# Genesis-Embodied-AI/ThinShellLab

Measured on AMD Instinct MI355X. Metric: element-steps/s (fwd+adjoint), 100k-tri cloth; 1/2/4/8-GPU scaling, higher is better.
Workload: dtype f64

## Files before the change

### thinshelllab_amd/csrc/k_cloth.hpp

```cpp
#pragma once
#include "tsl_ctx.hpp"
#include "tsl_device.hpp"

struct FaceGeom {
  d3 n;
  double h[3];
  double ca[3];
};

TSL_DEV FaceGeom face_geom(const d3 P[3]) {
  FaceGeom g;
  g.n = normalized(cross(P[1] - P[0], P[2] - P[1]));
#pragma unroll
  for (int l = 0; l < 3; l++) {
    const d3 p = P[l], a = P[(l + 1) % 3], b = P[(l + 2) % 3];
    const d3 en = cross(g.n, b - a);
    g.h[l] = fabs(dot(p - a, en)) / norm(en);
    g.ca[l] = dot(normalized(a - p), normalized(b - p));
  }
  return g;
}

TSL_DEV bool sign_neg(const d3& n2, const d3& e) { return dot(n2, e) < -1e-10 * norm(e); }
TSL_DEV double dihedral(const d3& n1, const d3& n2, const d3& e) {
// ... 384 lines not shown
            if (l != m) L[(m * 3 + j) * 9 + l * 3 + k] += Hlm[k * 3 + j];
          }
      }
  }

  if (CLAMP_ALL) spd_clamp<9>(L);
  double* R = rec + (size_t)t * 81;
#pragma unroll
  for (int l = 0; l < 3; l++)
#pragma unroll
    for (int m = 0; m < 3; m++)
#pragma unroll
      for (int j = 0; j < 3; j++)
#pragma unroll
        for (int k = 0; k < 3; k++) R[(l * 3 + m) * 9 + j * 3 + k] = L[(l * 3 + j) * 9 + m * 3 + k];
}

__global__ void __launch_bounds__(256) k_cloth_hess_hinge(ClothArgs A, const double* __restrict__ pos, double* __restrict__ rec) {
  const int h = blockIdx.x * blockDim.x + threadIdx.x;
  if (h >= A.n_hinge) return;
  const int f1 = A.hg_info[8 * h], l = A.hg_info[8 * h + 1], f2 = A.hg_info[8 * h + 2], p4 = A.hg_info[8 * h + 3], p21 = A.hg_info[8 * h + 4];
  const ClothDev c = A.cloth[A.cid[f1]];
  int v1[3], v2[3]; d3 P1[3], P2[3];
  load_face(pos, A.f2v, f1, v1, P1);
  load_face(pos, A.f2v, f2, v2, P2);
  const FaceGeom g1 = face_geom(P1), g2 = face_geom(P2);
  d3 g[4];
  hinge_grad(g1, g2, l, p4, p21, g);
  const double d2 = 2.0 * c.Kb * c.dx * c.dx * (1.0 / 3.0);
  double* R = rec + (size_t)h * 16;
#pragma unroll
  for (int j = 0; j < 4; j++) { R[3 * j] = g[j].x; R[3 * j + 1] = g[j].y; R[3 * j + 2] = g[j].z; }
  R[12] = d2;
}

#define CG_BPW 28
__global__ void __launch_bounds__(256) k_cloth_gather(int n_blk, const int* __restrict__ base, const int* __restrict__ ptr, const unsigned* __restrict__ ent, int n_hinge, int n_cface,
                                                      const double* __restrict__ hrec, const double* __restrict__ frec, const double* __restrict__ trec, double* __restrict__ vals) {
  __shared__ double tile[9][CG_BPW + 1];
  const int b0 = blockIdx.x * CG_BPW, t = threadIdx.x;
  if (t < 9 * CG_BPW) {
    const int bl = t / 9, e9 = t - 9 * bl, b = b0 + bl, r = e9 / 3, c = e9 - 3 * r;
    double acc = 0.0;
    if (b < n_blk) {
      for (int q = ptr[b]; q < ptr[b + 1]; q++) {
        const unsigned e = ent[q];
        const int el = (int)((e >> 4) & 0x7ffffff), pr = (int)(e & 15);
        if ((e >> 30) == 1) {
          acc += trec[(size_t)(el & 0x3ffffff) * 144 + pr * 9 + e9];
        } else if (e >> 31) {
          const int j = pr >> 2, k = pr & 3;
          const double* R = hrec + (size_t)el * 16;
          acc += R[12] * (R[3 * j + r] * R[3 * k + c]);
        } else {
          acc += frec[(size_t)el * 81 + pr * 9 + e9];
        }
      }
    }
    tile[e9][bl] = acc;
  }
  __syncthreads();
  if (t < 9 * CG_BPW) {
    const int e9 = t / CG_BPW, bl = t - CG_BPW * e9, b = b0 + bl;
    if (b < n_blk) vals[(size_t)base[b] + 64 * e9] += tile[e9][bl];
  }
}
// ... 14 lines not shown
```

### thinshelllab_amd/csrc/k_contact.hpp

```cpp
#pragma once

#include "k_solver.hpp"
#include "tsl_ctx.hpp"
#include "tsl_device.hpp"

struct ContactArgs {
  const int* idx;
  const double *w, *n, *dx0, *k, *mu, *T;
  double k_contact, eps_contact, eps_vh;
};

TSL_DEV double fr_f0(double x, double eh) { return (x > eh) ? x : (-x * x * x / (3.0 * eh * eh) + x * x / eh + eh / 3.0); }
TSL_DEV double fr_f1(double x, double eh) { return (x > eh) ? 1.0 / x : (-x / (eh * eh) + 2.0 / eh); }
TSL_DEV double fr_f2(double x, double eh) { return (x > eh) ? -1.0 / (x * x) : -1.0 / (eh * eh); }

__global__ void k_vn_gather(int NV, const int* __restrict__ ptr, const int* __restrict__ lst, const int* __restrict__ faces, const double* __restrict__ pos, double* __restrict__ vn) {
  const int i = blockIdx.x * blockDim.x + threadIdx.x;
  if (i >= NV) return;
  d3 a = d3();
  for (int e = ptr[i]; e < ptr[i + 1]; e++) {
    const int f = lst[e];
    const d3 v1 = ld3(pos, faces[3 * f]), v2 = ld3(pos, faces[3 * f + 1]), v3 = ld3(pos, faces[3 * f + 2]);
    a = a + cross(v2 - v1, v3 - v1);
  }
// ... 462 lines not shown

#define CONTACT_MV_THREADS 1024
TSL_DEV double contact_matvec_lane(int nc, const int* __restrict__ idx, const int* __restrict__ rowpos, const double* __restrict__ Hm, const double* __restrict__ x,
                                   double* __restrict__ y) {
  const int ci = blockIdx.x * 64 + (threadIdx.x >> 4);
  const int r = threadIdx.x & 15;
  if (ci >= nc || r >= 12) return 0.0;
  const double* H = Hm + 144 * (size_t)ci + 12 * r;
  double s = 0, xr = 0;
  int prr = 0;
#pragma unroll
  for (int k = 0; k < 4; k++) {
    const int pk = rowpos[idx[4 * ci + k]];
    const d3 v = ld3(x, pk);
    s += H[3 * k] * v.x + H[3 * k + 1] * v.y + H[3 * k + 2] * v.z;
    if (k == r / 3) { prr = pk; xr = (r % 3 == 0) ? v.x : (r % 3 == 1) ? v.y : v.z; }
  }
  if (s != 0.0) atomicAdd(&y[3 * (size_t)prr + (r % 3)], s);
  return s * xr;
}

__global__ void k_cr_count(int nc, const int* __restrict__ idx, const int* __restrict__ rowpos, int* __restrict__ cnt) {
  const int q = blockIdx.x * blockDim.x + threadIdx.x;
  if (q >= 4 * nc) return;
  atomicAdd(&cnt[rowpos[idx[q]]], 1);
}
__global__ void k_cr_fill(int nc, const int* __restrict__ idx, const int* __restrict__ rowpos, const int* __restrict__ ptr, int* __restrict__ fill, int* __restrict__ tmp) {
  const int q = blockIdx.x * blockDim.x + threadIdx.x;
  if (q >= 4 * nc) return;
  const int p = rowpos[idx[q]];
  tmp[ptr[p] + atomicAdd(&fill[p], 1)] = q;
}
__global__ void k_cr_rank(int nc, const int* __restrict__ idx, const int* __restrict__ rowpos, const int* __restrict__ ptr, const int* __restrict__ tmp, int* __restrict__ ent,
                          int4* __restrict__ rows) {
  const int q = blockIdx.x * blockDim.x + threadIdx.x;
  if (q >= 4 * nc) return;
  const int c4 = q & ~3;
  const int4 r = make_int4(rowpos[idx[c4]], rowpos[idx[c4 + 1]], rowpos[idx[c4 + 2]], rowpos[idx[c4 + 3]]);
  const int p = (q & 3) == 0 ? r.x : (q & 3) == 1 ? r.y : (q & 3) == 2 ? r.z : r.w;
  const int s0 = ptr[p], s1 = ptr[p + 1];
  int rank = 0;
  for (int e = s0; e < s1; e++) rank += tmp[e] < q ? 1 : 0;
  ent[s0 + rank] = q;
  rows[s0 + rank] = r;
}

__global__ void __launch_bounds__(CONTACT_MV_THREADS)
k_contact_matvec(int nc, const int* __restrict__ idx, const int* __restrict__ rowpos, const double* __restrict__ Hm, const double* __restrict__ x,
                 double* __restrict__ y, CgScal* sc, int slot, int check_flag) {
  if (check_flag && sc->flag) return;
  double acc = contact_matvec_lane(nc, idx, rowpos, Hm, x, y);
  if (slot >= 0) {
    acc = wave_sum(acc);
    if ((threadIdx.x & 63) == 0 && acc != 0.0) atomicAdd(&sc->pAp[slot], acc);
  }
}



__global__ void k_contact_backprop(int nc, ContactArgs A, const double* __restrict__ pos, const double* __restrict__ z, double* __restrict__ cg) {
  const int ci = blockIdx.x * blockDim.x + threadIdx.x;
  if (ci >= nc) return;
  int id[4];
  for (int k = 0; k < 4; k++) id[k] = A.idx[4 * ci + k];
  const d3 x0 = ld3(pos, id[0]), xa = ld3(pos, id[1]), xb = ld3(pos, id[2]), xp = ld3(pos, id[3]);
  const double w[3] = {A.w[3 * ci], A.w[3 * ci + 1], A.w[3 * ci + 2]};
  const double kf = A.k[ci];
  const double* T = A.T + 6 * (size_t)ci;
  const d3 x_c = x0 * w[0] + xa * w[1] + xb * w[2];
  const d3 dx = xp - x_c - ld3(A.dx0, ci);
  const double u[2] = {T[0] * dx.x + T[1] * dx.y + T[2] * dx.z, T[3] * dx.x + T[4] * dx.y + T[5] * dx.z};
  const double r = sqrt(u[0] * u[0] + u[1] * u[1]);
  const double f1 = fr_f1(r, A.eps_vh), f2 = fr_f2(r, A.eps_vh);
  const double pressure = kf / A.mu[ci];
  double g1[3];
  for (int j = 0; j < 3; j++) g1[j] = kf * f1 * (u[0] * T[j] + u[1] * T[3 + j]);
  const d3 n_c = ld3(A.n, ci);
// ... 566 lines not shown
    HIP_OK(hipMemcpyAsync(&n_ee, c->ee_qscan.p + QE, sizeof(int), hipMemcpyDeviceToHost, s));
    HIP_OK(hipMemcpyAsync(&big_edges, c->ee_nvf.p + 1, sizeof(int), hipMemcpyDeviceToHost, s));
  }
  int nc = 0, big_bucket = 0;
  if (Q > 0) HIP_OK(hipMemcpyAsync(&nc, c->cq_scan.p + Q, sizeof(int), hipMemcpyDeviceToHost, s));
  HIP_OK(hipMemcpyAsync(&big_bucket, c->nc_dev.p + 1, sizeof(int), hipMemcpyDeviceToHost, s));
  HIP_OK(hipStreamSynchronize(s));
  HIP_OK(hipGetLastError());
  if (big_bucket > 0) {
    c->nc = 0;
    return tsl_fail("contact detection: %d triangles of one body fall into one broad-phase cell (more than %d are not ranked): the body lies outside grid_extent = %g m "
                    "(centroids are clamped into the boundary cells) or grid_h = %g m is far larger than its triangles", big_bucket, TSL_BUCKET_CAP, c->grid_extent, c->grid_h);
  }
  if (big_edges > 0) {
    c->nc = 0;
    return tsl_fail("contact detection (contact_ee): %d surface-edge midpoints of one body fall into one broad-phase cell (more than %d are not ranked): the body lies "
                    "outside grid_extent = %g m or grid_h = %g m is far larger than its edges", big_edges, TSL_BUCKET_CAP, c->grid_extent, c->grid_h);
  }
  if (ee && (long)nc + n_ee > c->max_n_constraints) {
    c->nc = 0;
    return tsl_fail("contact detection: %d vertex-triangle + %d edge-edge active constraints exceed max_n_constraints = %d (raise the scene's max_n_constraints)", nc, n_ee,
                    c->max_n_constraints);
  }
  if (nc > c->max_n_constraints) {
    c->nc = 0;
    return tsl_fail("contact detection: %d active constraints exceed max_n_constraints = %d (raise the scene's max_n_constraints)", nc, c->max_n_constraints);
  }
  nc += n_ee;
  c->nc = nc; c->nc_ee = n_ee;
  if (nc_host) *nc_host = c->nc;
  if (c->nc > 0) {
    const int n1 = NV + 1;
    if (c->cr_ptr.n == 0) {
      if (c->cr_ptr.alloc(n1) | c->cr_cnt.alloc(n1) | c->cr_fill.alloc(n1) | c->cr_ent.alloc(4 * (size_t)c->max_n_constraints) | c->cr_rows.alloc(4 * (size_t)c->max_n_constraints) | c->cr_tmp.alloc(4 * (size_t)c->max_n_constraints)) return -1;
    }
    HIP_OK(hipMemsetAsync(c->cr_cnt.p, 0, n1 * sizeof(int), s));
    HIP_OK(hipMemsetAsync(c->cr_fill.p, 0, n1 * sizeof(int), s));
    hipLaunchKernelGGL(k_cr_count, dim3(cnblk(4 * (long)c->nc, 256)), dim3(256), 0, s, c->nc, c->c_idx.p, c->rowpos.p, c->cr_cnt.p);
    scan_exclusive(s, n1, c->cr_cnt.p, c->cr_ptr.p, c->scan_tmp.p);
    hipLaunchKernelGGL(k_cr_fill, dim3(cnblk(4 * (long)c->nc, 256)), dim3(256), 0, s, c->nc, c->c_idx.p, c->rowpos.p, (const int*)c->cr_ptr.p, c->cr_fill.p, c->cr_tmp.p);
    hipLaunchKernelGGL(k_cr_rank, dim3(cnblk(4 * (long)c->nc, 256)), dim3(256), 0, s, c->nc, c->c_idx.p, c->rowpos.p, (const int*)c->cr_ptr.p, (const int*)c->cr_tmp.p, c->cr_ent.p, c->cr_rows.p);
    HIP_OK(hipGetLastError());
  }
  return 0;
}

static ContactArgs ee_args(ContactArgs A, int nvf) {
  A.idx += 4 * (size_t)nvf; A.w += 3 * (size_t)nvf; A.n += 3 * (size_t)nvf; A.dx0 += 3 * (size_t)nvf; A.k += nvf; A.mu += nvf; A.T += 6 * (size_t)nvf;
  return A;
}

extern "C" int tsl_contact_counts(tsl_ctx* c, int32_t* out2) {
  if (!c || !out2) return tsl_fail("tsl_contact_counts: null argument");
  out2[0] = c->nc - c->nc_ee; out2[1] = c->nc_ee;
  return 0;
}

static bool direct_takes_solve(tsl_ctx* c);
static void contact_diag_refresh(tsl_ctx* c, hipStream_t s) {
  hipLaunchKernelGGL(k_contact_diag, dim3(cnblk((long)c->NV * 64, 256)), dim3(256), 0, s, c->NV, (const int*)c->cr_ptr.p, (const int*)c->cr_ent.p, (const double*)c->c_H.p, c->c_diag.p);
  c->cdiag_valid = true;
}
static int contact_assemble(tsl_ctx* c, const double* pos, int spd, double* grad, hipStream_t s) {
  if (c->nc <= 0) return 0;
  ContactArgs A;
  A.idx = c->c_idx.p; A.w = c->c_w.p; A.n = c->c_n.p; A.dx0 = c->c_dx0.p; A.k = c->c_k.p; A.mu = c->c_mu.p; A.T = c->c_T.p;
  A.k_contact = c->k_contact; A.eps_contact = c->eps_contact; A.eps_vh = c->eps_v * c->dt;
  if (grad && c->c_G.n < 12 * (size_t)c->max_n_constraints) { if (c->c_G.alloc(12 * (size_t)c->max_n_constraints)) return -1; }
  double* cg = grad ? c->c_G.p : (double*)nullptr;
  const int nvf = c->nc - c->nc_ee;
  if (nvf > 0) {
    if (c->spd_literal && spd == 1) hipLaunchKernelGGL(k_contact_assemble_coop<true>, dim3(cnblk((long)nvf * 16, 256)), dim3(256), 0, s, nvf, A, pos, spd, c->c_Hfull.p, cg);
    else hipLaunchKernelGGL(k_contact_assemble_coop<false>, dim3(cnblk((long)nvf * 16, 256)), dim3(256), 0, s, nvf, A, pos, spd, c->c_Hfull.p, cg);
  }
// ... 64 lines not shown
```

### thinshelllab_amd/csrc/tsl_ctx.hpp

```cpp
#pragma once
#include <memory>
#include <hip/hip_runtime.h>
#include <stdint.h>

#include <algorithm>
#include <cmath>
#include <cstdio>
#include <cstring>
#include <string>
#include <vector>

#include "../../include/tsl_hip.h"
#include "k_body.hpp"
#include "direct_plan.hpp"

#define TSL_SLICE 64

extern thread_local std::string g_tsl_err;
int tsl_fail(const char* fmt, ...);

#define HIP_OK(call)                                                                     \
  do {                                                                                   \
    hipError_t e__ = (call);                                                             \
    if (e__ != hipSuccess) return tsl_fail("%s failed: %s (%s:%d)", #call, hipGetErrorString(e__), __FILE__, __LINE__); \
// ... 259 lines not shown
  bool pc_separate = false, pc_frozen = false, in_step = false;
  bool cdiag_valid = false;
  bool dinv_valid = false;
  const double *st_pos = nullptr, *st_prev = nullptr, *st_vel = nullptr, *st_ref = nullptr;
  int fwd_spd_pc = 1;
  int adj_spd_pc = 1;
  DevBuf<SolverScalars> scal;
  DevBuf<double> part_pAp, part_rz, part_rr;
  SolverScalars* h_scal = nullptr;
  SolverScalars* h_scal2 = nullptr;
  hipEvent_t rb_event[2] = {nullptr, nullptr};
  hipStream_t side = 0;
  hipEvent_t ev_fork = nullptr, ev_fork0 = nullptr, ev_g2 = nullptr, ev_join = nullptr, ev_join2 = nullptr, ev_hh = nullptr, ev_gf = nullptr;
  hipStream_t side2 = 0;

  DevBuf<double> F, pdir, x1;

  int n_body = 0, n_pair = 0;
  std::vector<tsl_body> h_bodies;
  std::vector<tsl_contact_pair> h_pairs;
  std::vector<int> self_contact;
  DevBuf<int> faces;
  DevBuf<int> border;
  DevBuf<double> vn;
  DevBuf<int> proj_flag, proj_dir, proj_idx;
  DevBuf<double> proj_w;
  DevBuf<int> nc_dev;
  int nc = 0;
  DevBuf<int> c_idx;
  DevBuf<double> c_w, c_n, c_dx0, c_k, c_mu, c_T;
  DevBuf<int> cr_ptr, cr_cnt, cr_fill, cr_ent;
  DevBuf<int4> cr_rows;
  DevBuf<int> cr_tmp;
  DevBuf<int> c_kind;
  DevBuf<double> c_H;
  DevBuf<double> c_Hfull;
  DevBuf<double> c_diag;
  DevBuf<double> c_G;
  DevBuf<int> grid_key, grid_val, grid_key2, grid_val2, grid_range;
  DevBuf<int> vnf_ptr, vnf_lst;
  DevBuf<int> cq_flag, cq_scan;
  DevBuf<int> grid_scan;
  std::vector<size_t> gb_f0, gb_t0, gb_s0;
  DevBuf<int> grid_cnt, grid_ptr, grid_cur, scan_tmp;
  int grid_buckets_max = 0;
  int max_body_faces = 0;
  struct EeDesc { int pair, target, qoff, nq; };
  int contact_ee = 0, nc_ee = 0;
  std::vector<int> h_ee_e0;
  std::vector<EeDesc> ee_desc;
  std::vector<char> ee_target;
  long ee_qtot = 0;
  bool ee_ready = false;
  DevBuf<int> ee_edges, ee_qlist;
  DevBuf<int> ee_key, ee_val, ee_key2, ee_val2, ee_range, ee_bcnt, ee_bptr, ee_bcur, ee_bscan;
  std::vector<size_t> ee_f0, ee_t0, ee_s0;
  DevBuf<unsigned long long> ee_lmax;
  DevBuf<int> ee_qcnt, ee_qscan, ee_cand, ee_scan_tmp, ee_nvf;

  std::vector<MgCloth*> mg;
  int mg_enable = -1;
  double mg_omega = 0.0;
  int mg_pi_iters = 12;
  DevBuf<double> mg_omega0, mg_pi_part, mg_pi_norm;
  int mg_nu = 1, mg_coarse_sweeps = 8, mg_fuse = 1, mg_fuse_restrict = 1, mg_max_levels = 16, mg_coarse_exact = 1, mg_coarse_lag = 0, mg_dense_nodes = 64, mg_dense_auto = 1;
  double last_step_iters_per_solve = 0.0;
// ... 36 lines not shown
```

### thinshelllab_amd/csrc/tsl_hip.hip

```cpp
#include <stdarg.h>
#include <cctype>
#include <chrono>
#include <mutex>

#include <array>
#include <map>

#include "k_cloth.hpp"
#include "k_contact.hpp"
#include "k_fem.hpp"
#include "k_mg.hpp"
#include "k_param.hpp"
#include "k_solver.hpp"
#include "tsl_ctx.hpp"

thread_local std::string g_tsl_err;
int tsl_fail(const char* fmt, ...) {
  char buf[1024];
  va_list ap;
  va_start(ap, fmt);
  vsnprintf(buf, sizeof(buf), fmt, ap);
  va_end(ap);
  g_tsl_err = buf;
  return -1;
// ... 564 lines not shown
  hipStream_t s = c->stream;
  if (c->n_cface) hipLaunchKernelGGL(k_cloth_normals, dim3(nblk(c->n_cface, 256)), dim3(256), 0, s, c->n_cface, pos, c->cf_f2v.p, c->norm_dir.p);
  const int nmax = std::max(std::max(c->NV, c->n_cface), std::max(c->n_hinge, c->n_tet));
  const int nvf = c->nc - c->nc_ee;
  const int nb1 = nblk(nmax, 256), nb2 = nvf > 0 ? nblk(nvf, 64) : 0, nb3 = c->nc_ee > 0 ? nblk(c->nc_ee, 64) : 0;
  if (c->e_part.n < (size_t)nb1 + (size_t)nblk(c->max_n_constraints, 64) + 1) { if (c->e_part.alloc((size_t)nb1 + (size_t)nblk(c->max_n_constraints, 64) + 1)) return -1; }
  if (c->n_stvk > 0) hipLaunchKernelGGL(k_energy_stvk, dim3(nb1), dim3(256), 0, s, vert_args(c), cloth_args(c), tet_args(c), pos, prev, vel, ref, c->e_part.p, stvk_args(c));
  else hipLaunchKernelGGL(k_energy, dim3(nb1), dim3(256), 0, s, vert_args(c), cloth_args(c), tet_args(c), pos, prev, vel, ref, c->e_part.p);
  if (nb2 > 0) hipLaunchKernelGGL(k_contact_energy, dim3(nb2), dim3(64), 0, s, nvf, contact_args(c), pos, c->e_part.p + nb1);
  if (nb3 > 0) hipLaunchKernelGGL(k_ee_energy, dim3(nb3), dim3(64), 0, s, c->nc_ee, ee_args(contact_args(c), nvf), pos, c->e_part.p + nb1 + nb2);
  hipLaunchKernelGGL(k_energy_final, dim3(1), dim3(256), 0, s, nb1 + nb2 + nb3, (const double*)c->e_part.p, &SC(c)->energy);
  return 0;
}
static int energy_sync(tsl_ctx* c, const double* pos, const double* prev, const double* vel, const double* ref, double* E) {
  TSL_TRY(energy_async(c, pos, prev, vel, ref));
  HIP_OK(hipMemcpyAsync(&HSC(c)->energy, &SC(c)->energy, sizeof(double), hipMemcpyDeviceToHost, c->stream));
  HIP_OK(hipStreamSynchronize(c->stream));
  *E = HSC(c)->energy;
  return 0;
}

extern "C" int tsl_energy(tsl_ctx* c, const double* pos, const double* prev, const double* vel, const double* ref, double* E) {
  Scope scope(c);
  return energy_sync(c, pos, prev, vel, ref, E);
}

__global__ void k_vertex_gather(int NV, const int* __restrict__ vg_ptr, const int* __restrict__ vg_idx, const double* __restrict__ stage, int lo, int hi, double* __restrict__ F) {
  const int v = blockIdx.x * blockDim.x + threadIdx.x;
  if (v >= NV) return;
  d3 a = ld3(F, v);
  for (int e = vg_ptr[v]; e < vg_ptr[v + 1]; e++) { const int i = vg_idx[e]; if (i >= lo && i < hi) a = a + ld3(stage, i); }
  st3(F, v, a);
}
__global__ void __launch_bounds__(256) k_contact_row_gather(int NV, const int* __restrict__ rowpos, const int* __restrict__ cr_ptr, const int* __restrict__ cr_ent,
                                                            const double* __restrict__ cg, double* __restrict__ F) {
  const int v = (int)((blockIdx.x * (size_t)blockDim.x + threadIdx.x) >> 6), lane = threadIdx.x & 63;
  if (v >= NV) return;
  const int p = rowpos[v];
  const int r0 = cr_ptr[p], r1 = cr_ptr[p + 1];
  if (r1 <= r0) return;
  double a0 = 0, a1 = 0, a2 = 0;
  for (int e = r0 + lane; e < r1; e += 64) {
    const int q = cr_ent[e];
    const double* g = cg + 12 * (size_t)(q >> 2) + 3 * (q & 3);
    a0 += g[0]; a1 += g[1]; a2 += g[2];
  }
  a0 = wave_sum(a0); a1 = wave_sum(a1); a2 = wave_sum(a2);
  if (lane == 0) st3(F, v, ld3(F, v) + d3(a0, a1, a2));
}

static void cloth_grad_face_launch(tsl_ctx* c, hipStream_t s, const ClothArgs& CA, const double* pos) {
  if (c->n_stvk > 0) hipLaunchKernelGGL(k_cloth_grad_face<true>, dim3(nblk(c->n_cface, 256)), dim3(256), 0, s, CA, pos, stvk_args(c));
  else hipLaunchKernelGGL(k_cloth_grad_face<false>, dim3(nblk(c->n_cface, 256)), dim3(256), 0, s, CA, pos, stvk_args(c));
}
static void cloth_hess_face_launch(tsl_ctx* c, hipStream_t s, const ClothArgs& CA, const double* pos, const double* ref, int spd) {
  const dim3 g(nblk(c->n_cface, 128)), b(128);
  const StvkArgs S = stvk_args(c);
  const bool lit = c->spd_literal && spd == 1;
  if (c->n_stvk > 0) {
    if (spd == 2) hipLaunchKernelGGL((k_cloth_hess_face<true, false, true>), g, b, 0, s, CA, pos, ref, c->quirk.p, spd, c->cg_frec.p, S);
    else if (lit) hipLaunchKernelGGL((k_cloth_hess_face<false, true, true>), g, b, 0, s, CA, pos, ref, c->quirk.p, spd, c->cg_frec.p, S);
    else hipLaunchKernelGGL((k_cloth_hess_face<false, false, true>), g, b, 0, s, CA, pos, ref, c->quirk.p, spd, c->cg_frec.p, S);
  } else {
    if (spd == 2) hipLaunchKernelGGL((k_cloth_hess_face<true>), g, b, 0, s, CA, pos, ref, c->quirk.p, spd, c->cg_frec.p, S);
    else if (lit) hipLaunchKernelGGL((k_cloth_hess_face<false, true>), g, b, 0, s, CA, pos, ref, c->quirk.p, spd, c->cg_frec.p, S);
    else hipLaunchKernelGGL((k_cloth_hess_face<false>), g, b, 0, s, CA, pos, ref, c->quirk.p, spd, c->cg_frec.p, S);
  }
}

static int assemble_enqueue_early(tsl_ctx* c, const double* pos, const double* prev, const double* vel, const double* ref, int spd, double* grad, int tet_warm_flag);
static int assemble_enqueue(tsl_ctx* c, const double* pos, const double* prev, const double* vel, const double* ref, int spd, double* grad, int tet_warm_flag) {
  hipStream_t s = c->stream;
  const int NV = c->NV;
  if (c->nc > 0 || c->n_tet > 0) return assemble_enqueue_early(c, pos, prev, vel, ref, spd, grad, tet_warm_flag);
  HIP_OK(hipMemsetAsync(c->vals_full.p, 0, c->vals_full.n * sizeof(double), s));
  if (c->n_cface) hipLaunchKernelGGL(k_cloth_normals, dim3(nblk(c->n_cface, 256)), dim3(256), 0, s, c->n_cface, pos, c->cf_f2v.p, c->norm_dir.p);
  ClothArgs CA = cloth_args(c);
  const VertArgs VA = vert_args(c);
  CA.gstage = c->vg_stage.p;
  if (grad) {
    HIP_OK(hipMemsetAsync(grad, 0, 3 * (size_t)NV * sizeof(double), s));
    hipLaunchKernelGGL(k_vert_grad, dim3(nblk(NV, 256)), dim3(256), 0, s, VA, pos, prev, vel, grad);
  }
  hipLaunchKernelGGL(k_vert_hess, dim3(nblk(NV, 256)), dim3(256), 0, s, VA, c->diag_blk.p, c->vals_full.p);
  if (grad) {
    if (c->n_cface) cloth_grad_face_launch(c, s, CA, pos);
    if (c->n_hinge) hipLaunchKernelGGL(k_cloth_grad_hinge, dim3(nblk(c->n_hinge, 256)), dim3(256), 0, s, CA, pos, ref);
  }
  if (c->n_cface) {
    const int nq = (int)c->h_cloth.size() * 9;
    hipLaunchKernelGGL(k_cloth_quirk, dim3(nblk(nq, 64)), dim3(64), 0, s, CA, (int)c->h_cloth.size(), pos, ref, c->quirk.p);
    cloth_hess_face_launch(c, s, CA, pos, ref, spd);
  }
  if (c->n_hinge) hipLaunchKernelGGL(k_cloth_hess_hinge, dim3(nblk(c->n_hinge, 256)), dim3(256), 0, s, CA, pos, c->cg_hrec.p);
  if (c->n_cgblk_cloth > 0)
    hipLaunchKernelGGL(k_cloth_gather, dim3(nblk(c->n_cgblk_cloth, CG_BPW)), dim3(256), 0, s, c->n_cgblk_cloth, c->cg_base.p, c->cg_ptr.p, (const unsigned*)c->cg_ent.p, c->n_hinge, c->n_cface,
                       (const double*)c->cg_hrec.p, (const double*)c->cg_frec.p, (const double*)c->cg_trec.p, c->vals_full.p);
  if (grad) {
    hipLaunchKernelGGL(k_vertex_gather, dim3(nblk(NV, 256)), dim3(256), 0, s, NV, (const int*)c->vg_ptr.p, (const int*)c->vg_idx.p, (const double*)c->vg_stage.p, 0, c->vg_ns, grad);
    hipLaunchKernelGGL(k_mask_vec, dim3(gsz(3 * (size_t)NV)), dim3(256), 0, s, 3 * (size_t)NV, c->frozen.p, grad);
  }
  hipLaunchKernelGGL(k_mask_matrix, dim3(c->n_slices), dim3(256), 0, s, c->n_slices, c->slice_off.p, c->slice_len.p, c->colidx.p, c->fzmask.p, c->mdt2.p,
                     c->vals_full.p, c->vals.p, NV);
  if (!c->pc_frozen) {
    if (direct_takes_solve(c)) c->dinv_valid = false;
    else TSL_TRY(block_jacobi_refresh(c));
  }
  HIP_OK(hipGetLastError());
  return 0;
}

static int assemble_enqueue_early(tsl_ctx* c, const double* pos, const double* prev, const double* vel, const double* ref, int spd, double* grad, int tet_warm_flag) {
  hipStream_t s = c->stream, st = c->side;
  const bool fork_t = c->n_tet > 0 && c->nc > 0;
  hipStream_t stt = fork_t ? c->side2 : st;
  const int NV = c->NV;
  ClothArgs CA = cloth_args(c);
  const VertArgs VA = vert_args(c);
  TetArgs TA = tet_args(c);
  CA.gstage = c->vg_stage.p; TA.gstage = c->vg_stage.p + 3 * (size_t)c->vg_tet0;
  HIP_OK(hipEventRecord(c->ev_fork0, s));
  HIP_OK(hipStreamWaitEvent(st, c->ev_fork0, 0));
  if (fork_t) HIP_OK(hipStreamWaitEvent(stt, c->ev_fork0, 0));
  TSL_TRY(contact_assemble(c, pos, spd, grad, st));
  const bool gather = c->n_cgblk > 0;
  const bool hh_side = fork_t && gather;
  if (hh_side && c->n_hinge) {
    hipLaunchKernelGGL(k_cloth_hess_hinge, dim3(nblk(c->n_hinge, 256)), dim3(256), 0, stt, CA, pos, c->cg_hrec.p);
    HIP_OK(hipEventRecord(c->ev_hh, stt));
  }
  if (c->n_tet) {
    if (grad) { hipLaunchKernelGGL(k_tet_grad, dim3(nblk(c->n_tet, 256)), dim3(256), 0, stt, TA, pos); HIP_OK(hipEventRecord(c->ev_g2, stt)); }
    const bool lit = c->spd_literal && spd == 1;
    double* vws = (c->tet_warm && spd != 0 && !lit) ? c->tet_V.p : (double*)nullptr;
    if (lit) hipLaunchKernelGGL(k_tet_hess_coop<true>, dim3(nblk(c->n_tet, 16)), dim3(256), 0, stt, TA, pos, spd, vws, 0, c->cg_trec.p);
    else hipLaunchKernelGGL(k_tet_hess_coop<false>, dim3(nblk(c->n_tet, 16)), dim3(256), 0, stt, TA, pos, spd, vws, vws ? tet_warm_flag : 0, c->cg_trec.p);
  }
  HIP_OK(hipMemsetAsync(c->vals_full.p, 0, c->vals_full.n * sizeof(double), s));
  if (c->n_cface) hipLaunchKernelGGL(k_cloth_normals, dim3(nblk(c->n_cface, 256)), dim3(256), 0, s, c->n_cface, pos, c->cf_f2v.p, c->norm_dir.p);
  if (grad) {
    HIP_OK(hipMemsetAsync(grad, 0, 3 * (size_t)NV * sizeof(double), s));
    hipLaunchKernelGGL(k_vert_grad, dim3(nblk(NV, 256)), dim3(256), 0, s, VA, pos, prev, vel, grad);
  }
  hipLaunchKernelGGL(k_vert_hess, dim3(nblk(NV, 256)), dim3(256), 0, s, VA, c->diag_blk.p, c->vals_full.p);
  HIP_OK(hipEventRecord(c->ev_fork, s));
  if (c->n_cface) {
    const int nq = (int)c->h_cloth.size() * 9;
    hipLaunchKernelGGL(k_cloth_quirk, dim3(nblk(nq, 64)), dim3(64), 0, s, CA, (int)c->h_cloth.size(), pos, ref, c->quirk.p);
    cloth_hess_face_launch(c, s, CA, pos, ref, spd);
  }
  HIP_OK(hipStreamWaitEvent(stt, c->ev_fork, 0));
  if (c->n_hinge && !hh_side) hipLaunchKernelGGL(k_cloth_hess_hinge, dim3(nblk(c->n_hinge, 256)), dim3(256), 0, s, CA, pos, c->cg_hrec.p);
  const int nt_blk = c->n_cgblk - c->n_cgblk_cloth;
  if (c->n_tet && nt_blk > 0)
    hipLaunchKernelGGL(k_cloth_gather, dim3(nblk(nt_blk, CG_BPW)), dim3(256), 0, stt, nt_blk, c->cg_base.p + c->n_cgblk_cloth, c->cg_ptr.p + c->n_cgblk_cloth, (const unsigned*)c->cg_ent.p,
                       c->n_hinge, c->n_cface, (const double*)c->cg_hrec.p, (const double*)c->cg_frec.p, (const double*)c->cg_trec.p, c->vals_full.p);
  HIP_OK(hipEventRecord(c->ev_join2, stt));
  if (grad) {
    if (fork_t) HIP_OK(hipStreamWaitEvent(st, c->ev_fork, 0));
    if (c->n_hinge) hipLaunchKernelGGL(k_cloth_grad_hinge, dim3(nblk(c->n_hinge, 256)), dim3(256), 0, st, CA, pos, ref);
    if (c->n_cface) {
      cloth_grad_face_launch(c, hh_side ? stt : st, CA, pos);
      if (hh_side) HIP_OK(hipEventRecord(c->ev_gf, stt));
    }
  }
  if (hh_side && c->n_hinge) HIP_OK(hipStreamWaitEvent(s, c->ev_hh, 0));
  if (gather && c->n_cgblk_cloth > 0)
    hipLaunchKernelGGL(k_cloth_gather, dim3(nblk(c->n_cgblk_cloth, CG_BPW)), dim3(256), 0, s, c->n_cgblk_cloth, c->cg_base.p, c->cg_ptr.p, (const unsigned*)c->cg_ent.p, c->n_hinge, c->n_cface,
                       (const double*)c->cg_hrec.p, (const double*)c->cg_frec.p, (const double*)c->cg_trec.p, c->vals_full.p);
  HIP_OK(hipStreamWaitEvent(s, c->ev_join2, 0));
  hipLaunchKernelGGL(k_mask_matrix, dim3(c->n_slices), dim3(256), 0, s, c->n_slices, c->slice_off.p, c->slice_len.p, c->colidx.p, c->fzmask.p, c->mdt2.p,
                     c->vals_full.p, c->vals.p, NV);
  if (grad) {
    if (fork_t && c->n_tet) HIP_OK(hipStreamWaitEvent(st, c->ev_g2, 0));
    if (hh_side && c->n_cface) HIP_OK(hipStreamWaitEvent(st, c->ev_gf, 0));
    hipLaunchKernelGGL(k_vertex_gather, dim3(nblk(NV, 256)), dim3(256), 0, st, NV, (const int*)c->vg_ptr.p, (const int*)c->vg_idx.p, (const double*)c->vg_stage.p, 0, c->vg_ns, grad);
    if (c->nc > 0) hipLaunchKernelGGL(k_contact_row_gather, dim3(nblk((long)NV * 64, 256)), dim3(256), 0, st, NV, (const int*)c->rowpos.p, (const int*)c->cr_ptr.p, (const int*)c->cr_ent.p,
                                      (const double*)c->c_G.p, grad);
    hipLaunchKernelGGL(k_mask_vec, dim3(gsz(3 * (size_t)NV)), dim3(256), 0, st, 3 * (size_t)NV, c->frozen.p, grad);
  }
  HIP_OK(hipEventRecord(c->ev_join, st));
  HIP_OK(hipStreamWaitEvent(s, c->ev_join, 0));
  if (!c->pc_frozen) {
    if (direct_takes_solve(c)) c->dinv_valid = false;
    else TSL_TRY(block_jacobi_refresh(c));
  }
  HIP_OK(hipGetLastError());
  return 0;
}

static int assemble(tsl_ctx* c, const double* pos, const double* prev, const double* vel, const double* ref, int spd, double* grad) {
  hipStream_t s = c->stream;
  if (c->vg_stage.n < 3 * (size_t)std::max(c->vg_ns, 1)) { if (c->vg_stage.alloc(3 * (size_t)std::max(c->vg_ns, 1))) return tsl_fail("out of device memory (gradient staging)"); }
  if (c->n_tet > 0 && c->cg_trec.n < 144 * (size_t)c->n_tet) { if (c->cg_trec.alloc(144 * (size_t)c->n_tet)) return tsl_fail("out of device memory (element records)"); }
  if (grad && c->nc > 0 && c->c_G.n < 12 * (size_t)c->max_n_constraints) { if (c->c_G.alloc(12 * (size_t)c->max_n_constraints)) return -1; }
  if (c->n_cgblk > 0 && c->n_cface > 0 && c->cg_frec.n == 0) {
    if (c->cg_hrec.alloc((size_t)std::max(c->n_hinge, 1) * 16) | c->cg_frec.alloc((size_t)c->n_cface * 81)) return tsl_fail("out of device memory (cloth element records)");
  }
  int warm = 0;
  if (c->n_tet > 0 && c->tet_warm && spd != 0 && !(c->spd_literal && spd == 1)) {
    if (c->tet_V.n < (size_t)81 * c->n_tet) {
      if (c->tet_V.alloc((size_t)81 * c->n_tet)) return tsl_fail("out of device memory (tet eigenvectors)");
      HIP_OK(hipMemsetAsync(c->tet_V.p, 0, c->tet_V.n * sizeof(double), s));
      c->tet_V_count = 0;
    }
    warm = (c->tet_V_count++ % 16) != 0;
  }
  c->st_pos = pos; c->st_prev = prev; c->st_vel = vel; c->st_ref = ref;
  c->ds.numeric_valid = false;
  if (spd != c->ds.anorm_spd) { c->ds.anorm_valid = false; c->ds.anorm_spd = spd; }
  if (!c->pc_frozen) { c->mg_ops_valid = false; c->pc_separate = false; }
// ... 2018 lines not shown
  if (spd_pc) c->pc_separate = true;
  *rhs = pg_s;
  return 0;
}

static int adjoint_post(tsl_ctx* c, const AdjArgs& a) {
  hipStream_t s = c->stream;
  const int NV = c->NV;
  const size_t n3 = 3 * (size_t)NV, nr = 3 * (size_t)std::max(c->n_cface, 1);
  double* pg_s = a.pos_grad + (size_t)a.step * n3;
  double* pg_prev = a.pos_grad + (size_t)(a.step - 1) * n3;
  double* pg_prev2 = a.step > 1 ? a.pos_grad + (size_t)(a.step - 2) * n3 : nullptr;
  const double* x_s = a.pos_buffer + (size_t)a.step * n3;
  const double* x_prev = a.pos_buffer + (size_t)(a.step - 1) * n3;
  double* ag_s = a.angleref_grad + (size_t)a.step * nr;
  double* ag_prev = a.angleref_grad + (size_t)(a.step - 1) * nr;
  const double* ref_prev = a.ref_buffer + (size_t)(a.step - 1) * nr;
  (void)pg_s; (void)x_prev; (void)ag_s; (void)ref_prev;
  double* tmp_z_frozen = a.tmp_z_frozen;
  const double adj_damping = a.adj_damping;
  ClothArgs CA = cloth_args(c);
  hipLaunchKernelGGL(k_zfrozen_gather, dim3(nblk(NV, 256)), dim3(256), 0, s, NV, c->slice_off.p, c->slice_len.p, c->colidx.p, (const int*)c->trans.p, c->fzmask.p, c->vals_full.p,
                     c->v_x.p, c->v_t4.p);
  hipLaunchKernelGGL(k_scatter_perm, dim3(nblk(NV, 256)), dim3(256), 0, s, NV, c->perm.p, c->v_t4.p, tmp_z_frozen);
  if (c->nc > 0) {
    hipLaunchKernelGGL(k_contact_zfrozen_gather, dim3(nblk((long)NV * 64, 256)), dim3(256), 0, s, NV, (const int*)c->rowpos.p, (const int*)c->cr_ptr.p, (const int*)c->cr_ent.p, c->c_idx.p,
                       c->frozen.p, c->c_Hfull.p, c->pdir.p, tmp_z_frozen);
  }
  if (c->nc > 0) {
    if (c->c_G.n < 12 * (size_t)c->max_n_constraints) { if (c->c_G.alloc(12 * (size_t)c->max_n_constraints)) return -1; }
    const int nvf = c->nc - c->nc_ee;
    if (nvf > 0) hipLaunchKernelGGL(k_contact_backprop, dim3(nblk(nvf, 64)), dim3(64), 0, s, nvf, contact_args(c), x_s, c->pdir.p, c->c_G.p);
    if (c->nc_ee > 0) hipLaunchKernelGGL(k_ee_backprop, dim3(nblk(c->nc_ee, 64)), dim3(64), 0, s, c->nc_ee, ee_args(contact_args(c), nvf), x_s, c->pdir.p, c->c_G.p + 12 * (size_t)nvf);
    hipLaunchKernelGGL(k_contact_row_gather, dim3(nblk((long)NV * 64, 256)), dim3(256), 0, s, NV, (const int*)c->rowpos.p, (const int*)c->cr_ptr.p, (const int*)c->cr_ent.p,
                       (const double*)c->c_G.p, pg_prev);
  }
  if (c->n_hinge) hipLaunchKernelGGL(k_adj_x2a, dim3(nblk(c->n_hinge, 256)), dim3(256), 0, s, CA, x_s, c->pdir.p, ag_prev);
  hipLaunchKernelGGL(k_adj_prev, dim3(gsz(n3)), dim3(256), 0, s, NV, c->pdir.p, c->mass.p, c->frozen.p, c->dt, adj_damping, pg_prev, pg_prev2);
  HIP_OK(hipGetLastError());
  return 0;
}

extern "C" int tsl_adjoint_step(tsl_ctx* c, int step, int T, const double* pos_buffer, double* pos_grad, const double* ref_buffer, double* angleref_grad,
                                double* tmp_z_frozen, double adj_damping, tsl_solve_stats* st) {
  Scope scope(c);
  if (step < 1 || step >= T) return tsl_fail("tsl_adjoint_step: step %d outside [1, %d)", step, T);
  const AdjArgs a{step, T, pos_buffer, pos_grad, ref_buffer, angleref_grad, tmp_z_frozen, adj_damping};
  double* pg_s = nullptr;
  TSL_TRY(adjoint_pre(c, a, &pg_s));
  tsl_solve_stats local;
  if (!st) st = &local;
  TSL_TRY(solve_orig(c, pg_s, c->pdir.p, st));
  if (st->method == 4) TSL_TRY(direct_prezero(c));
  if (c->verbose) fprintf(stderr, "[tsl] adjoint step %d: nc %d solver flag %d iters %d restarts %d rel_residual %.2e\n", step, c->nc, st->flag, st->iters, st->restarts, st->rel_residual);
  TSL_TRY(adjoint_post(c, a));
  HIP_OK(hipStreamSynchronize(c->stream));
  HIP_OK(hipGetLastError());
  return 0;
}

extern "C" int tsl_group_adjoint_step(tsl_group* G, int step, int T, const double* const* pos_buffer_a, double* const* pos_grad_a, const double* const* ref_buffer_a,
                                      double* const* angleref_grad_a, double* const* tmp_z_a, const double* adj_damping_a, tsl_solve_stats* stats) {
  const int n = (int)G->m.size();
  tsl_ctx* g = G->g;
  if (step < 1 || step >= T) return tsl_fail("tsl_group_adjoint_step: step %d outside [1, %d)", step, T);
  std::vector<std::unique_ptr<Scope>> scopes;
  for (int i = 0; i < n; i++) scopes.emplace_back(new Scope(G->m[i]));
  std::vector<AdjArgs> aa(n);
// ... 32 lines not shown
```

Measured before the change: 530,900.

## Fuse hinge gradient into hinge Hessian kernel and gather contact rows by head list

A new combined hinge kernel computes the face geometry and hinge gradient once, then writes both the Hessian record and the staged bending gradient. This replaces separate grad and hess hinge launches, which each recomputed the same geometry. Contact row gather now launches one wave per contacted vertex, using a head list built during ranking, instead of one wave per mesh vertex. The cost is an extra event dependency in the gradient stream and a small head buffer. With many vertices but few contacts, far fewer idle waves are launched.

```diff
diff --git a/thinshelllab_amd/csrc/k_cloth.hpp b/thinshelllab_amd/csrc/k_cloth.hpp
--- a/thinshelllab_amd/csrc/k_cloth.hpp
+++ b/thinshelllab_amd/csrc/k_cloth.hpp
@@ -440,6 +440,28 @@
 #pragma unroll
   for (int j = 0; j < 4; j++) { R[3 * j] = g[j].x; R[3 * j + 1] = g[j].y; R[3 * j + 2] = g[j].z; }
   R[12] = d2;
+}
+
+__global__ void __launch_bounds__(256) k_cloth_hinge_both(ClothArgs A, const double* __restrict__ pos, const double* __restrict__ ref_angle, double* __restrict__ rec) {
+  const int h = blockIdx.x * blockDim.x + threadIdx.x;
+  if (h >= A.n_hinge) return;
+  const int f1 = A.hg_info[8 * h], l = A.hg_info[8 * h + 1], f2 = A.hg_info[8 * h + 2], p4 = A.hg_info[8 * h + 3], p21 = A.hg_info[8 * h + 4];
+  const ClothDev c = A.cloth[A.cid[f1]];
+  int v1[3], v2[3]; d3 P1[3], P2[3];
+  load_face(pos, A.f2v, f1, v1, P1);
+  load_face(pos, A.f2v, f2, v2, P2);
+  const FaceGeom g1 = face_geom(P1), g2 = face_geom(P2);
+  d3 g[4];
+  hinge_grad(g1, g2, l, p4, p21, g);
+  const double d2 = 2.0 * c.Kb * c.dx * c.dx * (1.0 / 3.0);
+  double* R = rec + (size_t)h * 16;
+#pragma unroll
+  for (int j = 0; j < 4; j++) { R[3 * j] = g[j].x; R[3 * j + 1] = g[j].y; R[3 * j + 2] = g[j].z; }
+  R[12] = d2;
+  const double theta = dihedral(g1.n, g2.n, ld3(pos, pick3(v1, (l + 1) % 2)) - ld3(pos, pick3(v1, l)));
+  const double dth = 2.0 * c.Kb * (theta - ref_angle[3 * f1 + l]) * c.dx * c.dx * (1.0 / 3.0);
+#pragma unroll
+  for (int j = 0; j < 4; j++) st3(A.gstage, A.gs_hinge + 4 * h + j, dth * g[j]);
 }
 
 #define CG_BPW 28
diff --git a/thinshelllab_amd/csrc/k_contact.hpp b/thinshelllab_amd/csrc/k_contact.hpp
--- a/thinshelllab_amd/csrc/k_contact.hpp
+++ b/thinshelllab_amd/csrc/k_contact.hpp
@@ -518,7 +518,7 @@
   tmp[ptr[p] + atomicAdd(&fill[p], 1)] = q;
 }
 __global__ void k_cr_rank(int nc, const int* __restrict__ idx, const int* __restrict__ rowpos, const int* __restrict__ ptr, const int* __restrict__ tmp, int* __restrict__ ent,
-                          int4* __restrict__ rows) {
+                          int4* __restrict__ rows, int* __restrict__ head) {
   const int q = blockIdx.x * blockDim.x + threadIdx.x;
   if (q >= 4 * nc) return;
   const int c4 = q & ~3;
@@ -529,6 +529,7 @@
   for (int e = s0; e < s1; e++) rank += tmp[e] < q ? 1 : 0;
   ent[s0 + rank] = q;
   rows[s0 + rank] = r;
+  head[q] = rank == 0 ? idx[q] : -1;
 }
 
 __global__ void __launch_bounds__(CONTACT_MV_THREADS)
@@ -1161,14 +1162,16 @@
   if (c->nc > 0) {
     const int n1 = NV + 1;
     if (c->cr_ptr.n == 0) {
-      if (c->cr_ptr.alloc(n1) | c->cr_cnt.alloc(n1) | c->cr_fill.alloc(n1) | c->cr_ent.alloc(4 * (size_t)c->max_n_constraints) | c->cr_rows.alloc(4 * (size_t)c->max_n_constraints) | c->cr_tmp.alloc(4 * (size_t)c->max_n_constraints)) return -1;
+      if (c->cr_ptr.alloc(n1) | c->cr_cnt.alloc(n1) | c->cr_fill.alloc(n1) | c->cr_ent.alloc(4 * (size_t)c->max_n_constraints) | c->cr_rows.alloc(4 * (size_t)c->max_n_constraints) | c->cr_tmp.alloc(4 * (size_t)c->max_n_constraints) |
+          c->cr_head.alloc(4 * (size_t)c->max_n_constraints)) return -1;
     }
     HIP_OK(hipMemsetAsync(c->cr_cnt.p, 0, n1 * sizeof(int), s));
     HIP_OK(hipMemsetAsync(c->cr_fill.p, 0, n1 * sizeof(int), s));
     hipLaunchKernelGGL(k_cr_count, dim3(cnblk(4 * (long)c->nc, 256)), dim3(256), 0, s, c->nc, c->c_idx.p, c->rowpos.p, c->cr_cnt.p);
     scan_exclusive(s, n1, c->cr_cnt.p, c->cr_ptr.p, c->scan_tmp.p);
     hipLaunchKernelGGL(k_cr_fill, dim3(cnblk(4 * (long)c->nc, 256)), dim3(256), 0, s, c->nc, c->c_idx.p, c->rowpos.p, (const int*)c->cr_ptr.p, c->cr_fill.p, c->cr_tmp.p);
-    hipLaunchKernelGGL(k_cr_rank, dim3(cnblk(4 * (long)c->nc, 256)), dim3(256), 0, s, c->nc, c->c_idx.p, c->rowpos.p, (const int*)c->cr_ptr.p, (const int*)c->cr_tmp.p, c->cr_ent.p, c->cr_rows.p);
+    hipLaunchKernelGGL(k_cr_rank, dim3(cnblk(4 * (long)c->nc, 256)), dim3(256), 0, s, c->nc, c->c_idx.p, c->rowpos.p, (const int*)c->cr_ptr.p, (const int*)c->cr_tmp.p, c->cr_ent.p, c->cr_rows.p,
+                       c->cr_head.p);
     HIP_OK(hipGetLastError());
   }
   return 0;
diff --git a/thinshelllab_amd/csrc/tsl_ctx.hpp b/thinshelllab_amd/csrc/tsl_ctx.hpp
--- a/thinshelllab_amd/csrc/tsl_ctx.hpp
+++ b/thinshelllab_amd/csrc/tsl_ctx.hpp
@@ -315,6 +315,7 @@
   DevBuf<int> cr_ptr, cr_cnt, cr_fill, cr_ent;
   DevBuf<int4> cr_rows;
   DevBuf<int> cr_tmp;
+  DevBuf<int> cr_head;
   DevBuf<int> c_kind;
   DevBuf<double> c_H;
   DevBuf<double> c_Hfull;
diff --git a/thinshelllab_amd/csrc/tsl_hip.hip b/thinshelllab_amd/csrc/tsl_hip.hip
--- a/thinshelllab_amd/csrc/tsl_hip.hip
+++ b/thinshelllab_amd/csrc/tsl_hip.hip
@@ -620,13 +620,14 @@
   for (int e = vg_ptr[v]; e < vg_ptr[v + 1]; e++) { const int i = vg_idx[e]; if (i >= lo && i < hi) a = a + ld3(stage, i); }
   st3(F, v, a);
 }
-__global__ void __launch_bounds__(256) k_contact_row_gather(int NV, const int* __restrict__ rowpos, const int* __restrict__ cr_ptr, const int* __restrict__ cr_ent,
-                                                            const double* __restrict__ cg, double* __restrict__ F) {
-  const int v = (int)((blockIdx.x * (size_t)blockDim.x + threadIdx.x) >> 6), lane = threadIdx.x & 63;
-  if (v >= NV) return;
+__global__ void __launch_bounds__(256) k_contact_row_gather(int n_head, const int* __restrict__ cr_head, const int* __restrict__ rowpos, const int* __restrict__ cr_ptr,
+                                                            const int* __restrict__ cr_ent, const double* __restrict__ cg, double* __restrict__ F) {
+  const int w = (int)((blockIdx.x * (size_t)blockDim.x + threadIdx.x) >> 6), lane = threadIdx.x & 63;
+  if (w >= n_head) return;
+  const int v = cr_head[w];
+  if (v < 0) return;
   const int p = rowpos[v];
   const int r0 = cr_ptr[p], r1 = cr_ptr[p + 1];
-  if (r1 <= r0) return;
   double a0 = 0, a1 = 0, a2 = 0;
   for (int e = r0 + lane; e < r1; e += 64) {
     const int q = cr_ent[e];
@@ -635,6 +636,11 @@
   }
   a0 = wave_sum(a0); a1 = wave_sum(a1); a2 = wave_sum(a2);
   if (lane == 0) st3(F, v, ld3(F, v) + d3(a0, a1, a2));
+}
+static void contact_row_gather_launch(tsl_ctx* c, hipStream_t s, const double* cg, double* F) {
+  const int n_head = 4 * c->nc;
+  hipLaunchKernelGGL(k_contact_row_gather, dim3(nblk((long)n_head * 64, 256)), dim3(256), 0, s, n_head, (const int*)c->cr_head.p, (const int*)c->rowpos.p, (const int*)c->cr_ptr.p,
+                     (const int*)c->cr_ent.p, cg, F);
 }
 
 static void cloth_grad_face_launch(tsl_ctx* c, hipStream_t s, const ClothArgs& CA, const double* pos) {
@@ -654,6 +660,11 @@
     else if (lit) hipLaunchKernelGGL((k_cloth_hess_face<false, true>), g, b, 0, s, CA, pos, ref, c->quirk.p, spd, c->cg_frec.p, S);
     else hipLaunchKernelGGL((k_cloth_hess_face<false>), g, b, 0, s, CA, pos, ref, c->quirk.p, spd, c->cg_frec.p, S);
   }
+}
+
+static void cloth_hinge_launch(tsl_ctx* c, hipStream_t s, const ClothArgs& CA, const double* pos, const double* ref, bool grad) {
+  if (grad) hipLaunchKernelGGL(k_cloth_hinge_both, dim3(nblk(c->n_hinge, 256)), dim3(256), 0, s, CA, pos, ref, c->cg_hrec.p);
+  else hipLaunchKernelGGL(k_cloth_hess_hinge, dim3(nblk(c->n_hinge, 256)), dim3(256), 0, s, CA, pos, c->cg_hrec.p);
 }
 
 static int assemble_enqueue_early(tsl_ctx* c, const double* pos, const double* prev, const double* vel, const double* ref, int spd, double* grad, int tet_warm_flag);
@@ -671,16 +682,13 @@
     hipLaunchKernelGGL(k_vert_grad, dim3(nblk(NV, 256)), dim3(256), 0, s, VA, pos, prev, vel, grad);
   }
   hipLaunchKernelGGL(k_vert_hess, dim3(nblk(NV, 256)), dim3(256), 0, s, VA, c->diag_blk.p, c->vals_full.p);
-  if (grad) {
-    if (c->n_cface) cloth_grad_face_launch(c, s, CA, pos);
-    if (c->n_hinge) hipLaunchKernelGGL(k_cloth_grad_hinge, dim3(nblk(c->n_hinge, 256)), dim3(256), 0, s, CA, pos, ref);
-  }
+  if (grad && c->n_cface) cloth_grad_face_launch(c, s, CA, pos);
   if (c->n_cface) {
     const int nq = (int)c->h_cloth.size() * 9;
     hipLaunchKernelGGL(k_cloth_quirk, dim3(nblk(nq, 64)), dim3(64), 0, s, CA, (int)c->h_cloth.size(), pos, ref, c->quirk.p);
     cloth_hess_face_launch(c, s, CA, pos, ref, spd);
   }
-  if (c->n_hinge) hipLaunchKernelGGL(k_cloth_hess_hinge, dim3(nblk(c->n_hinge, 256)), dim3(256), 0, s, CA, pos, c->cg_hrec.p);
+  if (c->n_hinge) cloth_hinge_launch(c, s, CA, pos, ref, grad != nullptr);
   if (c->n_cgblk_cloth > 0)
     hipLaunchKernelGGL(k_cloth_gather, dim3(nblk(c->n_cgblk_cloth, CG_BPW)), dim3(256), 0, s, c->n_cgblk_cloth, c->cg_base.p, c->cg_ptr.p, (const unsigned*)c->cg_ent.p, c->n_hinge, c->n_cface,
                        (const double*)c->cg_hrec.p, (const double*)c->cg_frec.p, (const double*)c->cg_trec.p, c->vals_full.p);
@@ -714,7 +722,7 @@
   const bool gather = c->n_cgblk > 0;
   const bool hh_side = fork_t && gather;
   if (hh_side && c->n_hinge) {
-    hipLaunchKernelGGL(k_cloth_hess_hinge, dim3(nblk(c->n_hinge, 256)), dim3(256), 0, stt, CA, pos, c->cg_hrec.p);
+    cloth_hinge_launch(c, stt, CA, pos, ref, grad != nullptr);
     HIP_OK(hipEventRecord(c->ev_hh, stt));
   }
   if (c->n_tet) {
@@ -738,7 +746,10 @@
     cloth_hess_face_launch(c, s, CA, pos, ref, spd);
   }
   HIP_OK(hipStreamWaitEvent(stt, c->ev_fork, 0));
-  if (c->n_hinge && !hh_side) hipLaunchKernelGGL(k_cloth_hess_hinge, dim3(nblk(c->n_hinge, 256)), dim3(256), 0, s, CA, pos, c->cg_hrec.p);
+  if (c->n_hinge && !hh_side) {
+    cloth_hinge_launch(c, s, CA, pos, ref, grad != nullptr);
+    if (grad) HIP_OK(hipEventRecord(c->ev_hh, s));
+  }
   const int nt_blk = c->n_cgblk - c->n_cgblk_cloth;
   if (c->n_tet && nt_blk > 0)
     hipLaunchKernelGGL(k_cloth_gather, dim3(nblk(nt_blk, CG_BPW)), dim3(256), 0, stt, nt_blk, c->cg_base.p + c->n_cgblk_cloth, c->cg_ptr.p + c->n_cgblk_cloth, (const unsigned*)c->cg_ent.p,
@@ -746,7 +757,6 @@
   HIP_OK(hipEventRecord(c->ev_join2, stt));
   if (grad) {
     if (fork_t) HIP_OK(hipStreamWaitEvent(st, c->ev_fork, 0));
-    if (c->n_hinge) hipLaunchKernelGGL(k_cloth_grad_hinge, dim3(nblk(c->n_hinge, 256)), dim3(256), 0, st, CA, pos, ref);
     if (c->n_cface) {
       cloth_grad_face_launch(c, hh_side ? stt : st, CA, pos);
       if (hh_side) HIP_OK(hipEventRecord(c->ev_gf, stt));
@@ -762,9 +772,9 @@
   if (grad) {
     if (fork_t && c->n_tet) HIP_OK(hipStreamWaitEvent(st, c->ev_g2, 0));
     if (hh_side && c->n_cface) HIP_OK(hipStreamWaitEvent(st, c->ev_gf, 0));
+    if (c->n_hinge) HIP_OK(hipStreamWaitEvent(st, c->ev_hh, 0));
     hipLaunchKernelGGL(k_vertex_gather, dim3(nblk(NV, 256)), dim3(256), 0, st, NV, (const int*)c->vg_ptr.p, (const int*)c->vg_idx.p, (const double*)c->vg_stage.p, 0, c->vg_ns, grad);
-    if (c->nc > 0) hipLaunchKernelGGL(k_contact_row_gather, dim3(nblk((long)NV * 64, 256)), dim3(256), 0, st, NV, (const int*)c->rowpos.p, (const int*)c->cr_ptr.p, (const int*)c->cr_ent.p,
-                                      (const double*)c->c_G.p, grad);
+    if (c->nc > 0) contact_row_gather_launch(c, st, (const double*)c->c_G.p, grad);
     hipLaunchKernelGGL(k_mask_vec, dim3(gsz(3 * (size_t)NV)), dim3(256), 0, st, 3 * (size_t)NV, c->frozen.p, grad);
   }
   HIP_OK(hipEventRecord(c->ev_join, st));
@@ -2849,8 +2859,7 @@
     const int nvf = c->nc - c->nc_ee;
     if (nvf > 0) hipLaunchKernelGGL(k_contact_backprop, dim3(nblk(nvf, 64)), dim3(64), 0, s, nvf, contact_args(c), x_s, c->pdir.p, c->c_G.p);
     if (c->nc_ee > 0) hipLaunchKernelGGL(k_ee_backprop, dim3(nblk(c->nc_ee, 64)), dim3(64), 0, s, c->nc_ee, ee_args(contact_args(c), nvf), x_s, c->pdir.p, c->c_G.p + 12 * (size_t)nvf);
-    hipLaunchKernelGGL(k_contact_row_gather, dim3(nblk((long)NV * 64, 256)), dim3(256), 0, s, NV, (const int*)c->rowpos.p, (const int*)c->cr_ptr.p, (const int*)c->cr_ent.p,
-                       (const double*)c->c_G.p, pg_prev);
+    contact_row_gather_launch(c, s, (const double*)c->c_G.p, pg_prev);
   }
   if (c->n_hinge) hipLaunchKernelGGL(k_adj_x2a, dim3(nblk(c->n_hinge, 256)), dim3(256), 0, s, CA, x_s, c->pdir.p, ag_prev);
   hipLaunchKernelGGL(k_adj_prev, dim3(gsz(n3)), dim3(256), 0, s, NV, c->pdir.p, c->mass.p, c->frozen.p, c->dt, adj_damping, pg_prev, pg_prev2);
```

New measurement: 512,700. 0.966x the previous value.
